# freshman97/LinTransUNet

Measured on AMD Instinct MI355X. Metric: 128^3 CT patches/sec (fwd+bwd), higher is better.
Workload: dtype bf16; 1 GPU; MaskTransUnet train step (fwd + 5-level loss + bwd), 128^3 single-channel patches, 2 per GPU, dropout 0.3, random-init weights; global_batch=2, parallelism=dp1, side_stream_concurrent=True, allreduce=none (1 rank)

## Files before the change

lintransunet_amd/csrc/conv_c16_ring.hip:

```cpp
#include "gemm_desc.h"
#include "lds_dma.h"

#define C16_PITCH 12
#define C16_HROWS 768
#define C16_HBUF (C16_HROWS * 32)
#define C16_STAGE (2 * C16_HBUF)
#define C16_BIAS (C16_STAGE + 4 * 4096)
#define C16_SMEM (C16_BIAS + 128)
#define C16_CENTER ((1 * 10 + 1) * C16_PITCH + 1)

template <bool FLIP>
__global__ void __launch_bounds__(256, 2) conv3_c16_ring_bf16_kernel(const HaloArgs a, int bricks) {
  extern __shared__ __attribute__((aligned(1024))) char smem[];
  const int tid = threadIdx.x, lane = tid & 63, wave = tid >> 6;
  const int li = lane & 31, lh = lane >> 5;
  const int nbh = (a.H + 3) / 4, nbw = (a.W + 7) / 8, nbd = (a.D + 7) / 8;
  const uint32_t lds0 = lds_addr(smem);
  const char* zsrc = reinterpret_cast<const char*>(ltu_zero_line) + (lane & 1) * 16;

  const int per = (bricks + (int)gridDim.x - 1) / (int)gridDim.x;
  const int b_first = (int)blockIdx.x * per;
  const int b_end = min(bricks, b_first + per);
  if (b_first >= b_end) return;

  bf16x8 wreg[27];
#pragma unroll
  for (int t = 0; t < 27; ++t) {
    uint4 v = make_uint4(0u, 0u, 0u, 0u);
    if (li < a.N) v = *reinterpret_cast<const uint4*>(reinterpret_cast<const uint16_t*>(a.w) + ((long long)li * 27 + t) * 16 + lh * 8);
    wreg[t] = __builtin_bit_cast(bf16x8, v);
  }
  const int prow = lane >> 1;
  const char* hbase[6];
  int hpos[6];
#pragma unroll
  for (int s = 0; s < 6; ++s) {
    const int row = (wave * 6 + s) * 32 + prow;
    const int hd = row % C16_PITCH, hw = (row / C16_PITCH) % 10, hh = row / (10 * C16_PITCH);
    const int c = ((lane & 1) ^ (hw & 1)) * 8;
    const bool s1 = c >= a.c0;
    const long long rel = ((long long)(hh - 1) * a.W + (hw - 1)) * a.D + (hd - 1);
    hbase[s] = s1 ? reinterpret_cast<const char*>(a.x1) + ((c - a.c0) + rel * a.lda1) * 2 : reinterpret_cast<const char*>(a.x0) + (c + rel * a.lda0) * 2;
    hpos[s] = hh | (hw << 8) | (hd << 16) | ((row < 6 * 10 * C16_PITCH && hd < 10 ? 1 : 0) << 24) | ((s1 ? 1 : 0) << 25);
  }
  struct Coord { int b, h0, w0, d0; };
  auto decompose = [&](int brick) {
    const Brick bk = split_brick(brick, nbh, nbw, nbd);
    return Coord{bk.b, bk.bh * 4, bk.bw * 8, bk.bd * 8};
  };
  auto advance = [&](Coord c) {
    c.d0 += 8;
    if (c.d0 >= nbd * 8) {
      c.d0 = 0; c.w0 += 8;
      if (c.w0 >= nbw * 8) {
        c.w0 = 0; c.h0 += 4;
        if (c.h0 >= nbh * 4) { c.h0 = 0; c.b += 1; }
      }
    }
    return c;
  };
  auto issue_halo = [&](const Coord& cc, int buf) {
    const int b = cc.b, h0 = cc.h0, w0 = cc.w0, d0 = cc.d0;
    const long long vox0 = (((long long)b * a.H + h0) * a.W + w0) * a.D + d0;
    const long long off0 = vox0 * a.lda0 * 2, off1 = vox0 * a.lda1 * 2;
    const uint32_t hb = lds0 + buf * C16_HBUF + wave * 6 * 1024;
    if (h0 >= 1 && h0 + 5 <= a.H && w0 >= 1 && w0 + 9 <= a.W && d0 >= 1 && d0 + 9 <= a.D) {
#pragma unroll
      for (int s = 0; s < 6; ++s) {
        const char* src = ((hpos[s] >> 24) & 1) ? hbase[s] + (((hpos[s] >> 25) & 1) ? off1 : off0) : zsrc;
        glds16(src, hb + s * 1024);
      }
      return;
    }
#pragma unroll
    for (int s = 0; s < 6; ++s) {
      const int h = h0 - 1 + (hpos[s] & 255), w = w0 - 1 + ((hpos[s] >> 8) & 255), d = d0 - 1 + ((hpos[s] >> 16) & 255);
      const bool in = ((hpos[s] >> 24) & 1) != 0 && (unsigned)h < (unsigned)a.H && (unsigned)w < (unsigned)a.W && (unsigned)d < (unsigned)a.D;
      const char* src = in ? hbase[s] + (((hpos[s] >> 25) & 1) ? off1 : off0) : zsrc;
      glds16(src, hb + s * 1024);
    }
  };

  const int hwl = li >> 3;
  int baseA[2][3];
#pragma unroll
  for (int i = 0; i < 2; ++i) {
    const int row0 = ((wave + 1) * 10 + (i * 4 + hwl + 1)) * C16_PITCH + (li & 7) + 1;
#pragma unroll
    for (int dwi = 0; dwi < 3; ++dwi) baseA[i][dwi] = (row0 - C16_CENTER) * 32 + ((lh ^ ((hwl + dwi) & 1)) << 4);
  }

  if (tid < 32) reinterpret_cast<float*>(smem + C16_BIAS)[tid] = (a.bias != nullptr && tid < a.N) ? a.bias[tid] : 0.f;
  char* obase[4];
  int opos[4];
#pragma unroll
  for (int it = 0; it < 4; ++it) {
    const int idx = it * 64 + lane, vox = idx >> 2, part = idx & 3;
    const int n = part * 8;
    const bool d1 = n >= a.n0;
    const long long rel = (long long)(vox >> 3) * a.D + (vox & 7);
    obase[it] = d1 ? reinterpret_cast<char*>(a.o1) + ((n - a.n0) + rel * a.ldo1) * 2 : reinterpret_cast<char*>(a.o0) + (n + rel * a.ldo0) * 2;
    opos[it] = (vox >> 3) | ((vox & 7) << 8) | ((n < a.N ? 1 : 0) << 16) | ((d1 ? 1 : 0) << 17);
  }
  char* const stage = smem + C16_STAGE + wave * 4096;

  auto store_brick = [&](const Coord& cc) {
    const int b = cc.b, h0 = cc.h0, w0 = cc.w0, d0 = cc.d0;
    const long long vox0 = ((((long long)b * a.H + h0 + wave) * a.W + w0) * a.D + d0);
    const long long off0 = vox0 * a.ldo0 * 2, off1 = vox0 * a.ldo1 * 2;
    const bool hok = h0 + wave < a.H;
    const bool whole = w0 + 8 <= a.W && d0 + 8 <= a.D;
#pragma unroll
    for (int it = 0; it < 4; ++it) {
      const int idx = it * 64 + lane, vox = idx >> 2, part = idx & 3;
      const uint4 v = *reinterpret_cast<const uint4*>(stage + vox * 64 + ((part ^ ((vox >> 1) & 3)) << 4));
      const int ow = opos[it] & 255, od = (opos[it] >> 8) & 255;
      if (hok && ((opos[it] >> 16) & 1) != 0 && (whole || (w0 + ow < a.W && d0 + od < a.D)))
        *reinterpret_cast<uint4*>(obase[it] + (((opos[it] >> 17) & 1) ? off1 : off0)) = v;
    }
  };
  Coord cur = decompose(b_first), prev = cur, next = advance(cur);
  issue_halo(cur, 0);
  int buf = 0;
  for (int brick = b_first; brick < b_end; ++brick) {
    ring_sync<0>();
    if (brick > b_first) store_brick(prev);
    if (brick + 1 < b_end) issue_halo(next, buf ^ 1);
    prev = cur; cur = next; next = advance(next);
    const int hoff = buf * C16_HBUF;
    int bA[2][3];
#pragma unroll
    for (int i = 0; i < 2; ++i)
#pragma unroll
      for (int dwi = 0; dwi < 3; ++dwi) bA[i][dwi] = baseA[i][dwi] + hoff;
    f32x16 acc[2];
#pragma unroll
    for (int i = 0; i < 2; ++i)
#pragma unroll
      for (int r = 0; r < 16; ++r) acc[i][r] = 0.f;
    auto load_frags = [&](auto TT, bf16x8 (&af)[2]) {
      constexpr int t = decltype(TT)::value;
      constexpr int th = t / 9, tw = (t / 3) % 3, td = t % 3;
      constexpr int dh = FLIP ? 1 - th : th - 1, dw = FLIP ? 1 - tw : tw - 1, dd = FLIP ? 1 - td : td - 1;
      constexpr int immA = (((dh * 10 + dw) * C16_PITCH + dd) + C16_CENTER) * 32;
#pragma unroll
      for (int i = 0; i < 2; ++i) af[i] = *reinterpret_cast<const bf16x8*>(smem + bA[i][dw + 1] + immA);
    };
    bf16x8 afA[2], afB[2];
    load_frags(std::integral_constant<int, 0>{}, afA);
    static_for<0, 14>([&](auto TP) {
      constexpr int t = decltype(TP)::value * 2;
      if constexpr (t + 1 < 27) load_frags(std::integral_constant<int, t + 1>{}, afB);
      __builtin_amdgcn_sched_barrier(0);
#pragma unroll
      for (int i = 0; i < 2; ++i) acc[i] = __builtin_amdgcn_mfma_f32_32x32x16_bf16(wreg[t], afA[i], acc[i], 0, 0, 0);
      __builtin_amdgcn_sched_barrier(0);
      if constexpr (t + 2 < 27) load_frags(std::integral_constant<int, t + 2>{}, afA);
      __builtin_amdgcn_sched_barrier(0);
      if constexpr (t + 1 < 27) {
#pragma unroll
        for (int i = 0; i < 2; ++i) acc[i] = __builtin_amdgcn_mfma_f32_32x32x16_bf16(wreg[t + 1], afB[i], acc[i], 0, 0, 0);
      }
      __builtin_amdgcn_sched_barrier(0);
    });
#pragma unroll
    for (int rr = 0; rr < 4; ++rr) {
      const float4 bv = *reinterpret_cast<const float4*>(smem + C16_BIAS + (8 * rr + 4 * lh) * 4);
#pragma unroll
      for (int i = 0; i < 2; ++i) {
        const int vox = i * 32 + li;
        uint2 pk;
        pk.x = pack_bf16x2(acc[i][4 * rr + 0] + bv.x, acc[i][4 * rr + 1] + bv.y);
        pk.y = pack_bf16x2(acc[i][4 * rr + 2] + bv.z, acc[i][4 * rr + 3] + bv.w);
        *reinterpret_cast<uint2*>(stage + vox * 64 + ((rr ^ ((vox >> 1) & 3)) << 4) + lh * 8) = pk;
      }
    }
    buf ^= 1;
  }
  store_brick(prev);
}

int launch_conv_c16_ring_bf16(const HaloArgs& a, hipStream_t st) {
  if (a.C != 16 || a.N > 32 || a.N % 8 || a.n0 % 8 || a.c0 % 8 || a.lda0 % 8 || a.lda1 % 8 || a.ldo0 % 8 || a.ldo1 % 8) return 1;
  if (a.H < 2 || a.W < 4 || a.D < 4 || a.part != nullptr) return 1;
  const long long bricks = (long long)a.B * ((a.H + 3) / 4) * ((a.W + 7) / 8) * ((a.D + 7) / 8);
  if (bricks >= (1LL << 31) || bricks < 128) return 1;
  static LtuDevOnce attr_once;
  if (attr_once.first()) {
    ltu_dyn_lds(&conv3_c16_ring_bf16_kernel<false>, C16_SMEM);
    ltu_dyn_lds(&conv3_c16_ring_bf16_kernel<true>, C16_SMEM);
  }
  const int want = ltu_knob_pos("LTU_C16_RING_BLOCKS", 512);
  const int nblk = (int)(bricks < want ? bricks : want);
  if (a.flip) hipLaunchKernelGGL(conv3_c16_ring_bf16_kernel<true>, dim3(nblk), dim3(256), C16_SMEM, st, a, (int)bricks);
  else hipLaunchKernelGGL(conv3_c16_ring_bf16_kernel<false>, dim3(nblk), dim3(256), C16_SMEM, st, a, (int)bricks);
  return ltu_check_launch();
}
```

lintransunet_amd/csrc/conv_halo.hip:

```cpp
#include "gemm_desc.h"
#include "lds_dma.h"

#define HALO_H 6
#define HALO_W 6
#define HALO_D 10
#define HALO_VOX (HALO_H * HALO_W * HALO_D)
#define LDH 40

template <int WN, int TN, int TS>
constexpr int halo_smem_bytes() {
  constexpr int BN = WN * TN * 32;
  constexpr int be = HALO_VOX * 32 + 2 * TS * BN * LDH, se = 128 * (BN + 8);
  return 2 * (be > se ? be : se);
}
template <int WM, int WN, int TM, int TN, int TS, int CC>
__global__ void __launch_bounds__(256) conv3_halo_bf16_kernel(const HaloArgs a) {
  static_assert(WM * TM == 4 && WM * WN == 4, "128-row brick on 4 waves");
  constexpr int BN = WN * TN * 32, NSTAGE = 27 / TS;
  constexpr int VPV = CC / 8, KS = CC / 16;
  constexpr int PD = CC == 16 ? 12 : HALO_D, VMASK = VPV - 1;
  constexpr int HALO_ELEMS = HALO_VOX * 32, B_ELEMS = 2 * TS * BN * LDH, LDC = BN + 8, STAGE_ELEMS = 128 * LDC;
  extern __shared__ __attribute__((aligned(16))) uint16_t smem[];
  uint16_t* halo = smem;
  uint16_t* Bs = smem + HALO_ELEMS;
// ... 565 lines not shown
      const float4 q = *reinterpret_cast<const float4*>(a.part + ((long long)z * M + v) * a.N + n);
      acc.x += q.x; acc.y += q.y; acc.z += q.z; acc.w += q.w;
    }
    uint2 pk;
    pk.x = pack_bf16x2(acc.x, acc.y);
    pk.y = pack_bf16x2(acc.z, acc.w);
    uint16_t* dst = n < a.n0 ? reinterpret_cast<uint16_t*>(a.o0) + v * a.ldo0 + n
                             : reinterpret_cast<uint16_t*>(a.o1) + v * a.ldo1 + (n - a.n0);
    *reinterpret_cast<uint2*>(dst) = pk;
  }
}

static int halo_split(long long bricks, int N, int C, int CC, int* cps) {
  if (N <= 32 && C <= 32) return 1;
  const int ntn = (N > 64 && bricks * cdiv(N, 128) >= 256) ? cdiv(N, 128) : (N > 32 ? cdiv(N, 64) : 1);
  const long long blocks = bricks * ntn;
  const int nchunk = (C + CC - 1) / CC;
  if (blocks >= ltu_knob_pos("LTU_HALO_SPLIT_BELOW", 200) || nchunk < 2) return 1;
  int want = (int)((512 + blocks - 1) / blocks);
  if (want > 8) want = 8;
  if (want > nchunk) want = nchunk;
  if (want < 2) return 1;
  *cps = (nchunk + want - 1) / want;
  return (nchunk + *cps - 1) / *cps;
}
static int halo_cc(int C, int c0) { return (C % 32 == 0 && c0 % 32 == 0) ? 32 : 16; }
long long conv_halo_ws_floats(int B, int H, int W, int D, int C, int N) {
  const long long bricks = (long long)B * ((H + 3) / 4) * ((W + 3) / 4) * ((D + 7) / 8);
  int cps = 0;
  if (conv_ring_splits(B, H, W, D, C, N)) return 8LL * B * H * W * D * N;
  const int ks = halo_split(bricks, N, C, halo_cc(C, C), &cps);
  return (ks > 1 || halo_split(bricks, N, C, 16, &cps) > 1) ? 8LL * B * H * W * D * N : 0;
}

int launch_conv_halo_bf16(HaloArgs a, hipStream_t st) {
  if (a.C % 8 || a.c0 % 8 || a.lda0 % 8 || a.lda1 % 8 || a.N % 4 || a.n0 % 4 || a.ldo0 % 4 || a.ldo1 % 4) return 1;
  if (a.H < 2 || a.W < 2 || a.D < 4) return 1;
  a.CC = (a.C % 32 == 0 && a.c0 % 32 == 0) ? 32 : 16;
  if (a.C % 16 != 0 && a.C != 8) return 1;
  if (a.c0 % a.CC != 0 && a.c0 != a.C) return 1;
  const long long bricks = (long long)a.B * ((a.H + 3) / 4) * ((a.W + 3) / 4) * ((a.D + 7) / 8);
  if (bricks >= (1LL << 31)) return 1;
#ifdef LTU_EXPERIMENTS
  a.no_xcd_order = ltu_knob("LTU_HALO_NO_XCD", 0);
#else
  a.no_xcd_order = 0;
#endif
  if (a.C == 32 && a.N <= 32 && !ltu_knob("LTU_NO_FC_RING", 0)) {
    const int hr = launch_conv_fc_ring_bf16(a, st);
    if (hr != 1) return hr;
  }
  if (a.C == 16 && a.N <= 32 && !ltu_knob("LTU_NO_C16_RING", 0)) {
    const int hr = launch_conv_c16_ring_bf16(a, st);
    if (hr != 1) return hr;
  }
  if (a.N <= 32 && a.C <= 32 && !ltu_knob("LTU_NO_HALO_WS", 0)) {
    int wsb = -1;
    wsb = ltu_knob_pos("LTU_HALO_WS_BLOCKS", 512);
    const unsigned nblk = (unsigned)(bricks < wsb ? bricks : wsb);
    if (ltu_knob("LTU_HALO_WR", a.C <= 16 ? 1 : 0)) {
      const int wrb = ltu_knob_pos("LTU_HALO_WR_BLOCKS", a.C > 16 ? 256 : 512);
      const unsigned nb = (unsigned)(bricks < wrb ? bricks : wrb);
      if (a.C > 16) hipLaunchKernelGGL((conv3_halo_wr_bf16_kernel<32>), dim3(nb), dim3(256), 0, st, a, (int)bricks);
      else hipLaunchKernelGGL((conv3_halo_wr_bf16_kernel<16>), dim3(nb), dim3(256), 0, st, a, (int)bricks);
      return ltu_check_launch();
    }
    if (a.C > 16) hipLaunchKernelGGL((conv3_halo_ws_bf16_kernel<32>), dim3(nblk), dim3(256), 0, st, a, (int)bricks);
    else hipLaunchKernelGGL((conv3_halo_ws_bf16_kernel<16>), dim3(nblk), dim3(256), 0, st, a, (int)bricks);
    return ltu_check_launch();
  }
  if ((a.C >= 64 || a.N > 32) && !ltu_knob("LTU_NO_CONV_RING", 0)) {
    a.ksplit = 1;
    const int hr = launch_conv_ring_bf16(a, st);
    if (hr == LTU_OK && a.ksplit > 1) {
      const long long M = (long long)a.B * a.H * a.W * a.D;
      long long blocks = (M * (a.N / 4) + 255) / 256;
      if (blocks > 2048) blocks = 2048;
      hipLaunchKernelGGL(conv_halo_fold_kernel, dim3((unsigned)blocks), dim3(256), 0, st, a, M);
      return ltu_check_launch();
    }
    if (hr != 1) return hr;
  }
  int cps = 0;
  a.ksplit = a.part != nullptr && !ltu_knob("LTU_NO_HALO_SPLIT", 0) ? halo_split(bricks, a.N, a.C, a.CC, &cps) : 1;
  a.cps = cps;
  if (a.ksplit < 2) a.part = nullptr;
  else if ((long long)a.ksplit * a.B * a.H * a.W * a.D * a.N > a.part_floats) return LTU_E_ARG;
  const unsigned gz = (unsigned)a.ksplit;
  const int chunks_per_wg = a.ksplit > 1 ? a.cps : (a.C + a.CC - 1) / a.CC;
  const bool deep = ltu_knob("LTU_HALO_DEEP", chunks_per_wg >= 4 ? 1 : 0) != 0;
#define HALO_LAUNCH1(WM, WN, TM, TN, TS, CCV)                                                                        \
  do {                                                                                                               \
    auto kern = &conv3_halo_bf16_kernel<WM, WN, TM, TN, TS, CCV>;                                                    \
    constexpr int bytes = halo_smem_bytes<WN, TN, TS>();                                                            \
    static LtuDevOnce once;                                                                                          \
    if (once.first()) ltu_dyn_lds(kern, bytes);                                                                      \
    hipLaunchKernelGGL(kern, grid, dim3(256), bytes, st, a);                                                         \
  } while (0)
#define HALO_LAUNCH(WM, WN, TM, TN, TS)                     \
  do {                                                      \
    if (a.CC == 32) HALO_LAUNCH1(WM, WN, TM, TN, TS, 32);   \
    else HALO_LAUNCH1(WM, WN, TM, TN, TS, 16);              \
  } while (0)
  if (a.N > 64 && bricks * cdiv(a.N, 128) >= 256) {
    dim3 grid((unsigned)bricks, cdiv(a.N, 128), gz);
    if (deep) HALO_LAUNCH(2, 2, 2, 2, 3);
// ... 791 lines not shown
```

lintransunet_amd/csrc/gemm.hip:

```cpp
#include <stdlib.h>

#include "gemm_desc.h"

template <typename TA>
__device__ __forceinline__ float4 gather_a(const IGemmArgs& g, bool row_ok, const RowCoord& rc, int k) {
  float4 z = make_float4(0.f, 0.f, 0.f, 0.f);
  if (!row_ok || k >= g.K) return z;
  const int slot = k / g.C;
  const int c = k - slot * g.C;
  const Tap tp = g.tap[slot];
  int h = rc.h * g.mh + tp.dh, w = rc.w * g.mw + tp.dw, d = rc.d * g.md + tp.dd;
  if ((unsigned)h >= (unsigned)g.sh || (unsigned)w >= (unsigned)g.sw || (unsigned)d >= (unsigned)g.sd) return z;
  int ph = g.sh, pw = g.sw, pd = g.sd;
  if (g.ups) {
    h >>= 1; w >>= 1; d >>= 1;
    ph >>= 1; pw >>= 1; pd >>= 1;
  }
  const long long vox = (((long long)rc.b * ph + h) * pw + w) * pd + d;
  if (c < g.c0) return Vec4<TA>::load(reinterpret_cast<const TA*>(g.a0) + vox * g.lda0 + c);
  return Vec4<TA>::load(reinterpret_cast<const TA*>(g.a1) + vox * g.lda1 + (c - g.c0));
}

__device__ __forceinline__ float4 gather_w(const IGemmArgs& g, int n, int k) {
  if (n >= g.N || k >= g.K) return make_float4(0.f, 0.f, 0.f, 0.f);
// ... 410 lines not shown
                                      ltu_stream_t s) {
  if (dtype != LTU_BF16) return LTU_E_DTYPE;
  const int rc = launch_tn_ring_group_bf16(jobs, njobs, blocks, ws, ws_floats, (hipStream_t)s);
  return rc == 1 ? LTU_E_SHAPE : rc;
}

static bool use_halo() {
  int v = -1;
  v = ltu_knob("LTU_NO_HALO", 0) ? 0 : 1;
  return v == 1;
}

static int conv_fwd_desc(IGemmArgs& g, int B, int Hi, int Wi, int Di, int C0, int C1, int Co, int sh, int sw, int sd,
                         int ups, int* Ho, int* Wo, int* Do) {
  if ((sh != 1 && sh != 2) || (sw != 1 && sw != 2) || (sd != 1 && sd != 2)) return LTU_E_ARG;
  if (C0 % 4 != 0 || C1 % 4 != 0 || C0 <= 0) return LTU_E_SHAPE;
  memset(&g, 0, sizeof(g));
  const int Hl = ups ? 2 * Hi : Hi, Wl = ups ? 2 * Wi : Wi, Dl = ups ? 2 * Di : Di;
  *Ho = (Hl - 1) / sh + 1; *Wo = (Wl - 1) / sw + 1; *Do = (Dl - 1) / sd + 1;
  g.nb = B; g.rh = *Ho; g.rw = *Wo; g.rd = *Do;
  g.M = (long long)B * g.rh * g.rw * g.rd;
  g.N = Co; g.C = C0 + C1; g.c0 = C0; g.K = 27 * g.C;
  g.lda0 = C0; g.lda1 = C1;
  g.nseg = 1; g.wrow = 27 * g.C;
  g.sh = Hl; g.sw = Wl; g.sd = Dl; g.ups = ups ? 1 : 0;
  g.mh = sh; g.mw = sw; g.md = sd;
  g.ntaps = 27;
  for (int t = 0; t < 27; ++t) g.tap[t] = Tap{(int8_t)(t / 9 - 1), (int8_t)((t / 3) % 3 - 1), (int8_t)(t % 3 - 1), (int8_t)t};
  g.out_identity = 1;
  g.n0 = Co;
  return LTU_OK;
}

extern "C" int ltu_conv3d_fwd(const void* x0, const void* x1, const void* wf, const float* bias, void* y, int B, int Hi,
                              int Wi, int Di, int C0, int C1, int Co, int sh, int sw, int sd, int ups, float* ws, long long ws_floats,
                              int dtype, ltu_stream_t s) {
  IGemmArgs g;
  int Ho, Wo, Do;
  int rc = conv_fwd_desc(g, B, Hi, Wi, Di, C0, C1, Co, sh, sw, sd, ups, &Ho, &Wo, &Do);
  if (rc) return rc;
  g.a0 = x0; g.a1 = x1 ? x1 : x0;
  g.w[0] = wf; g.bias[0] = bias;
  g.o0 = y; g.o1 = y; g.ldo0 = Co; g.ldo1 = Co;
  if (dtype == LTU_BF16) {
    if (sh == 1 && sw == 1 && sd == 1 && !ups && use_halo()) {
      HaloArgs a;
      memset(&a, 0, sizeof(a));
      a.x0 = x0; a.x1 = x1 ? x1 : x0; a.w = wf; a.bias = bias; a.o0 = y; a.o1 = y;
      a.B = B; a.H = Hi; a.W = Wi; a.D = Di;
      a.C = C0 + C1; a.c0 = C0; a.lda0 = C0; a.lda1 = C1 > 0 ? C1 : C0;
      a.N = Co; a.n0 = Co; a.ldo0 = Co; a.ldo1 = Co;
      a.part = ws; a.part_floats = ws_floats;
      const int hr = launch_conv_halo_bf16(a, (hipStream_t)s);
      if (hr != 1) return hr;
    }
    g.part = ws; g.part_floats = ws_floats;
    return launch_nt_bf16(g, (hipStream_t)s);
  }
  if (dtype != LTU_F32) return LTU_E_DTYPE;
  return launch_nt<float, float>(g, (hipStream_t)s);
}

extern "C" long long ltu_conv3d_ws_floats(int B, int H, int W, int D, int C, int Co) {
  const long long halo = conv_halo_ws_floats(B, H, W, D, C, Co), ig = igemm_nt_ws_floats((long long)B * H * W * D, Co, 27 * C);
  return halo > ig ? halo : ig;
}
extern "C" long long ltu_igemm_ws_floats(long long M, int N, int K) { return igemm_nt_ws_floats(M, N, K); }

extern "C" int ltu_conv3d_wgrad(const void* grad, const void* x0, const void* x1, float* dwf, float* db, int B, int Hi,
                                int Wi, int Di, int C0, int C1, int Co, int sh, int sw, int sd, int ups, int torch_co,
                                int torch_ci, float* ws, long long ws_floats, int dtype, ltu_stream_t s) {
  WGradArgs wa;
  memset(&wa, 0, sizeof(wa));
  int Ho, Wo, Do;
  int rc = conv_fwd_desc(wa.g, B, Hi, Wi, Di, C0, C1, Co, sh, sw, sd, ups, &Ho, &Wo, &Do);
  if (rc) return rc;
  if (Co % 4 != 0) return LTU_E_SHAPE;
  wa.g.a0 = x0; wa.g.a1 = x1 ? x1 : x0;
  wa.grad = grad; wa.ldg = Co; wa.dw = dwf; wa.db = db; wa.t_co = torch_co; wa.t_ci = torch_ci;
  wa.part = dtype == LTU_BF16 ? ws : nullptr; wa.part_floats = ws_floats; wa.nseg_w = 1;
  if (dtype == LTU_BF16 && ws != nullptr && sh == 1 && sw == 1 && sd == 1 && !ups && use_halo()) {
    WHaloArgs h;
    memset(&h, 0, sizeof(h));
    h.x0 = x0; h.x1 = x1 ? x1 : x0; h.grad = grad;
    h.B = B; h.H = Hi; h.W = Wi; h.D = Di;
    h.C = C0 + C1; h.c0 = C0; h.lda0 = C0; h.lda1 = C1 > 0 ? C1 : C0;
    h.N = Co; h.ldg = Co; h.part = ws; h.part_floats = ws_floats;
    int nsplit = 0;
    const int hr = launch_conv_wgrad_halo_bf16(h, &nsplit, (hipStream_t)s);
    if (hr == LTU_OK) {
      wa.npad = Co; wa.kpad = 27 * (C0 + C1);
      wa.bpart = ws + (long long)nsplit * wa.npad * wa.kpad;
      return launch_wgrad_reduce(wa, nsplit, (hipStream_t)s);
    }
    if (hr != 1) return hr;
  }
  if (dtype == LTU_BF16) return launch_tn_bf16(wa, (hipStream_t)s);
  if (dtype != LTU_F32) return LTU_E_DTYPE;
  return launch_tn<float>(wa, (hipStream_t)s);
}

extern "C" int ltu_conv3d_dgrad(const void* grad, const void* wd, void* dx0, void* dx1, int B, int Hl, int Wl, int Dl,
                                int C0, int C1, int Co, int sh, int sw, int sd, float* ws, long long ws_floats, int dtype, ltu_stream_t s) {
  if ((sh != 1 && sh != 2) || (sw != 1 && sw != 2) || (sd != 1 && sd != 2)) return LTU_E_ARG;
  if (Co % 4 != 0) return LTU_E_SHAPE;
  if (dtype == LTU_BF16 && sh == 1 && sw == 1 && sd == 1 && use_halo()) {
// ... 210 lines not shown
```

lintransunet_amd/csrc/gemm_desc.h:

```cpp
#pragma once
#include <stdlib.h>
#include "common.h"

struct Tap {
  int8_t dh, dw, dd, wt;
};

struct IGemmArgs {
  const void* a0;
  const void* a1;
  const void* w[3];
  const float* bias[3];
  void* o0;
  void* o1;
  long long M;
  int N, K;
  int C, c0;
  int lda0, lda1;
  int nseg;
  int wrow;
  int nb, rh, rw, rd;
  int sh, sw, sd, ups;
  int mh, mw, md;
  int ntaps;
// ... 51 lines not shown

struct TnGeom {
  int bn, bk, nn, nk, rows, nsplit;
  long long ws_floats;
};
static inline TnGeom tn_geometry(long long M, int N, int K, int brows) {
  TnGeom t;
  t.bk = 128;
  t.bn = N > 64 ? 128 : (N > 32 ? 64 : 32);
  t.nk = (K + t.bk - 1) / t.bk;
  t.nn = (N + t.bn - 1) / t.bn;
  int tn_want = -1, tn_min = -1;
  tn_want = ltu_knob_pos("LTU_TN_WANT", 1024);
  tn_min = ltu_knob_pos("LTU_TN_MINROWS", 128);
  long long want = tn_want / ((long long)t.nk * t.nn);
  if (want < 1) want = 1;
  long long rows = (M + want - 1) / want;
  if (rows < tn_min) rows = tn_min;
  rows = (rows + brows - 1) / brows * brows;
  t.rows = (int)rows;
  t.nsplit = (int)((M + rows - 1) / rows);
  t.ws_floats = (long long)t.nsplit * t.nn * t.bn * ((long long)t.nk * t.bk + 1);
  return t;
}


int launch_nt_bf16(const IGemmArgs& g, hipStream_t st);
int launch_tn_bf16(WGradArgs& wa, hipStream_t st);

struct HaloArgs {
  const void* x0;
  const void* x1;
  const void* w;
  const float* bias;
  void* o0;
  void* o1;
  int B, H, W, D;
  int C, c0, lda0, lda1;
  int N, n0, ldo0, ldo1;
  int flip;
  int CC;
  float* part;
  long long part_floats;
  int ksplit, cps;
  int no_xcd_order;
};
long long conv_halo_ws_floats(int B, int H, int W, int D, int C, int N);
int launch_conv_halo_bf16(HaloArgs a, hipStream_t st);
bool conv_ring_splits(int B, int H, int W, int D, int C, int N);
int launch_conv_ring_bf16(HaloArgs& a, hipStream_t st);
int launch_conv_fc_ring_bf16(const HaloArgs& a, hipStream_t st);
int launch_conv_c16_ring_bf16(const HaloArgs& a, hipStream_t st);

struct WHaloArgs {
  const void* x0;
  const void* x1;
  const void* grad;
  const void* grad1;
  int gn0, ldg1;
  int B, H, W, D;
  int C, c0, lda0, lda1;
  int N, ldg;
  int CC;
  int bricks, bricks_per_split;
  float* part;
  long long part_floats;
  float* bpart;
  int npad, kpad;
};
long long conv_wgrad_halo_ws_floats(int N, int K);
int launch_conv_wgrad_halo_bf16(WHaloArgs a, int* nsplit_out, hipStream_t st);
int launch_conv_wgrad_halo_ring_bf16(WHaloArgs a, int* nsplit_out, hipStream_t st);
int launch_wgrad_reduce(const WGradArgs& wa, int nsplit, hipStream_t st);

bool tn_ring_shape_ok(long long M, int N, int K);
long long tn_ring_ws_floats(long long M, int N, int K);
int launch_tn_ring_bf16(WGradArgs& wa, hipStream_t st, int* nsplit_out = nullptr);
int launch_nt_ring_bf16(const IGemmArgs& g, hipStream_t st);
long long tn_ring_group_ws_floats(const ltu_wgrad_job* jobs, int njobs, int blocks);
int launch_tn_ring_group_bf16(const ltu_wgrad_job* jobs, int njobs, int blocks, float* ws, long long ws_floats, hipStream_t st);

struct ClsEntry {
  int8_t dh, dw, dd, cls;
  int wbase;
};
struct ClassHaloArgs {
  const void* x;
  const void* w;
  const float* bias;
  void* o0;
  void* o1;
  int B, H, W, D;
  int C, lda;
  int N, n0, ldo0, ldo1;
  int Hh, Wh, Dh;
  int mh, mw, md;
  int wrow;
  int nent, ncls;
  int cls_begin[9];
  int8_t cls_p[8][4];
  ClsEntry ent[64];
};
int launch_conv_class_halo_bf16(const ClassHaloArgs& a, hipStream_t st);
int launch_pw_small_bf16(const void* x, int lda, const void* w, const float* bias, void* y, int ldy, long long M, int N, int K, int accumulate,
                         hipStream_t st);
int launch_sdgrad_ring_bf16(const void* grad, const void* wd, void* dx, int B, int Hl, int Wl, int Dl, int N, int Co, int sd, hipStream_t st);
// ... 19 lines not shown
```

Baseline: 162.2 patches/s.

## Generalize C16 ring conv into template; add C8 and stride-(2,2,1) ring kernels

Moves the 16-channel ring-buffered halo conv kernel into a templated header parameterized by channel count and stride. The template is then used for two new kernels: an 8-channel stride-1 conv that packs two taps per MFMA k-slice, and a 16-channel stride-(2,2,1) forward conv. The aim is to move these layer shapes off the generic halo/workspace and implicit-GEMM paths onto the LDS-DMA double-buffered ring kernel. The trade-offs are more templated kernel code and new dispatch conditions, with the new paths taken only above a minimum brick count.

```diff
diff --git a/lintransunet_amd/csrc/conv_c16_ring.hip b/lintransunet_amd/csrc/conv_c16_ring.hip
--- a/lintransunet_amd/csrc/conv_c16_ring.hip
+++ b/lintransunet_amd/csrc/conv_c16_ring.hip
@@ -1,183 +1,11 @@
-#include "gemm_desc.h"
-#include "lds_dma.h"
+#include "conv_ring488.h"
 
-#define C16_PITCH 12
-#define C16_HROWS 768
-#define C16_HBUF (C16_HROWS * 32)
-#define C16_STAGE (2 * C16_HBUF)
-#define C16_BIAS (C16_STAGE + 4 * 4096)
-#define C16_SMEM (C16_BIAS + 128)
-#define C16_CENTER ((1 * 10 + 1) * C16_PITCH + 1)
+#define C16_SMEM (Ring488<16, 1>::SMEM)
 
 template <bool FLIP>
 __global__ void __launch_bounds__(256, 2) conv3_c16_ring_bf16_kernel(const HaloArgs a, int bricks) {
   extern __shared__ __attribute__((aligned(1024))) char smem[];
-  const int tid = threadIdx.x, lane = tid & 63, wave = tid >> 6;
-  const int li = lane & 31, lh = lane >> 5;
-  const int nbh = (a.H + 3) / 4, nbw = (a.W + 7) / 8, nbd = (a.D + 7) / 8;
-  const uint32_t lds0 = lds_addr(smem);
-  const char* zsrc = reinterpret_cast<const char*>(ltu_zero_line) + (lane & 1) * 16;
-
-  const int per = (bricks + (int)gridDim.x - 1) / (int)gridDim.x;
-  const int b_first = (int)blockIdx.x * per;
-  const int b_end = min(bricks, b_first + per);
-  if (b_first >= b_end) return;
-
-  bf16x8 wreg[27];
-#pragma unroll
-  for (int t = 0; t < 27; ++t) {
-    uint4 v = make_uint4(0u, 0u, 0u, 0u);
-    if (li < a.N) v = *reinterpret_cast<const uint4*>(reinterpret_cast<const uint16_t*>(a.w) + ((long long)li * 27 + t) * 16 + lh * 8);
-    wreg[t] = __builtin_bit_cast(bf16x8, v);
-  }
-  const int prow = lane >> 1;
-  const char* hbase[6];
-  int hpos[6];
-#pragma unroll
-  for (int s = 0; s < 6; ++s) {
-    const int row = (wave * 6 + s) * 32 + prow;
-    const int hd = row % C16_PITCH, hw = (row / C16_PITCH) % 10, hh = row / (10 * C16_PITCH);
-    const int c = ((lane & 1) ^ (hw & 1)) * 8;
-    const bool s1 = c >= a.c0;
-    const long long rel = ((long long)(hh - 1) * a.W + (hw - 1)) * a.D + (hd - 1);
-    hbase[s] = s1 ? reinterpret_cast<const char*>(a.x1) + ((c - a.c0) + rel * a.lda1) * 2 : reinterpret_cast<const char*>(a.x0) + (c + rel * a.lda0) * 2;
-    hpos[s] = hh | (hw << 8) | (hd << 16) | ((row < 6 * 10 * C16_PITCH && hd < 10 ? 1 : 0) << 24) | ((s1 ? 1 : 0) << 25);
-  }
-  struct Coord { int b, h0, w0, d0; };
-  auto decompose = [&](int brick) {
-    const Brick bk = split_brick(brick, nbh, nbw, nbd);
-    return Coord{bk.b, bk.bh * 4, bk.bw * 8, bk.bd * 8};
-  };
-  auto advance = [&](Coord c) {
-    c.d0 += 8;
-    if (c.d0 >= nbd * 8) {
-      c.d0 = 0; c.w0 += 8;
-      if (c.w0 >= nbw * 8) {
-        c.w0 = 0; c.h0 += 4;
-        if (c.h0 >= nbh * 4) { c.h0 = 0; c.b += 1; }
-      }
-    }
-    return c;
-  };
-  auto issue_halo = [&](const Coord& cc, int buf) {
-    const int b = cc.b, h0 = cc.h0, w0 = cc.w0, d0 = cc.d0;
-    const long long vox0 = (((long long)b * a.H + h0) * a.W + w0) * a.D + d0;
-    const long long off0 = vox0 * a.lda0 * 2, off1 = vox0 * a.lda1 * 2;
-    const uint32_t hb = lds0 + buf * C16_HBUF + wave * 6 * 1024;
-    if (h0 >= 1 && h0 + 5 <= a.H && w0 >= 1 && w0 + 9 <= a.W && d0 >= 1 && d0 + 9 <= a.D) {
-#pragma unroll
-      for (int s = 0; s < 6; ++s) {
-        const char* src = ((hpos[s] >> 24) & 1) ? hbase[s] + (((hpos[s] >> 25) & 1) ? off1 : off0) : zsrc;
-        glds16(src, hb + s * 1024);
-      }
-      return;
-    }
-#pragma unroll
-    for (int s = 0; s < 6; ++s) {
-      const int h = h0 - 1 + (hpos[s] & 255), w = w0 - 1 + ((hpos[s] >> 8) & 255), d = d0 - 1 + ((hpos[s] >> 16) & 255);
-      const bool in = ((hpos[s] >> 24) & 1) != 0 && (unsigned)h < (unsigned)a.H && (unsigned)w < (unsigned)a.W && (unsigned)d < (unsigned)a.D;
-      const char* src = in ? hbase[s] + (((hpos[s] >> 25) & 1) ? off1 : off0) : zsrc;
-      glds16(src, hb + s * 1024);
-    }
-  };
-
-  const int hwl = li >> 3;
-  int baseA[2][3];
-#pragma unroll
-  for (int i = 0; i < 2; ++i) {
-    const int row0 = ((wave + 1) * 10 + (i * 4 + hwl + 1)) * C16_PITCH + (li & 7) + 1;
-#pragma unroll
-    for (int dwi = 0; dwi < 3; ++dwi) baseA[i][dwi] = (row0 - C16_CENTER) * 32 + ((lh ^ ((hwl + dwi) & 1)) << 4);
-  }
-
-  if (tid < 32) reinterpret_cast<float*>(smem + C16_BIAS)[tid] = (a.bias != nullptr && tid < a.N) ? a.bias[tid] : 0.f;
-  char* obase[4];
-  int opos[4];
-#pragma unroll
-  for (int it = 0; it < 4; ++it) {
-    const int idx = it * 64 + lane, vox = idx >> 2, part = idx & 3;
-    const int n = part * 8;
-    const bool d1 = n >= a.n0;
-    const long long rel = (long long)(vox >> 3) * a.D + (vox & 7);
-    obase[it] = d1 ? reinterpret_cast<char*>(a.o1) + ((n - a.n0) + rel * a.ldo1) * 2 : reinterpret_cast<char*>(a.o0) + (n + rel * a.ldo0) * 2;
-    opos[it] = (vox >> 3) | ((vox & 7) << 8) | ((n < a.N ? 1 : 0) << 16) | ((d1 ? 1 : 0) << 17);
-  }
-  char* const stage = smem + C16_STAGE + wave * 4096;
-
-  auto store_brick = [&](const Coord& cc) {
-    const int b = cc.b, h0 = cc.h0, w0 = cc.w0, d0 = cc.d0;
-    const long long vox0 = ((((long long)b * a.H + h0 + wave) * a.W + w0) * a.D + d0);
-    const long long off0 = vox0 * a.ldo0 * 2, off1 = vox0 * a.ldo1 * 2;
-    const bool hok = h0 + wave < a.H;
-    const bool whole = w0 + 8 <= a.W && d0 + 8 <= a.D;
-#pragma unroll
-    for (int it = 0; it < 4; ++it) {
-      const int idx = it * 64 + lane, vox = idx >> 2, part = idx & 3;
-      const uint4 v = *reinterpret_cast<const uint4*>(stage + vox * 64 + ((part ^ ((vox >> 1) & 3)) << 4));
-      const int ow = opos[it] & 255, od = (opos[it] >> 8) & 255;
-      if (hok && ((opos[it] >> 16) & 1) != 0 && (whole || (w0 + ow < a.W && d0 + od < a.D)))
-        *reinterpret_cast<uint4*>(obase[it] + (((opos[it] >> 17) & 1) ? off1 : off0)) = v;
-    }
-  };
-  Coord cur = decompose(b_first), prev = cur, next = advance(cur);
-  issue_halo(cur, 0);
-  int buf = 0;
-  for (int brick = b_first; brick < b_end; ++brick) {
-    ring_sync<0>();
-    if (brick > b_first) store_brick(prev);
-    if (brick + 1 < b_end) issue_halo(next, buf ^ 1);
-    prev = cur; cur = next; next = advance(next);
-    const int hoff = buf * C16_HBUF;
-    int bA[2][3];
-#pragma unroll
-    for (int i = 0; i < 2; ++i)
-#pragma unroll
-      for (int dwi = 0; dwi < 3; ++dwi) bA[i][dwi] = baseA[i][dwi] + hoff;
-    f32x16 acc[2];
-#pragma unroll
-    for (int i = 0; i < 2; ++i)
-#pragma unroll
-      for (int r = 0; r < 16; ++r) acc[i][r] = 0.f;
-    auto load_frags = [&](auto TT, bf16x8 (&af)[2]) {
-      constexpr int t = decltype(TT)::value;
-      constexpr int th = t / 9, tw = (t / 3) % 3, td = t % 3;
-      constexpr int dh = FLIP ? 1 - th : th - 1, dw = FLIP ? 1 - tw : tw - 1, dd = FLIP ? 1 - td : td - 1;
-      constexpr int immA = (((dh * 10 + dw) * C16_PITCH + dd) + C16_CENTER) * 32;
-#pragma unroll
-      for (int i = 0; i < 2; ++i) af[i] = *reinterpret_cast<const bf16x8*>(smem + bA[i][dw + 1] + immA);
-    };
-    bf16x8 afA[2], afB[2];
-    load_frags(std::integral_constant<int, 0>{}, afA);
-    static_for<0, 14>([&](auto TP) {
-      constexpr int t = decltype(TP)::value * 2;
-      if constexpr (t + 1 < 27) load_frags(std::integral_constant<int, t + 1>{}, afB);
-      __builtin_amdgcn_sched_barrier(0);
-#pragma unroll
-      for (int i = 0; i < 2; ++i) acc[i] = __builtin_amdgcn_mfma_f32_32x32x16_bf16(wreg[t], afA[i], acc[i], 0, 0, 0);
-      __builtin_amdgcn_sched_barrier(0);
-      if constexpr (t + 2 < 27) load_frags(std::integral_constant<int, t + 2>{}, afA);
-      __builtin_amdgcn_sched_barrier(0);
-      if constexpr (t + 1 < 27) {
-#pragma unroll
-        for (int i = 0; i < 2; ++i) acc[i] = __builtin_amdgcn_mfma_f32_32x32x16_bf16(wreg[t + 1], afB[i], acc[i], 0, 0, 0);
-      }
-      __builtin_amdgcn_sched_barrier(0);
-    });
-#pragma unroll
-    for (int rr = 0; rr < 4; ++rr) {
-      const float4 bv = *reinterpret_cast<const float4*>(smem + C16_BIAS + (8 * rr + 4 * lh) * 4);
-#pragma unroll
-      for (int i = 0; i < 2; ++i) {
-        const int vox = i * 32 + li;
-        uint2 pk;
-        pk.x = pack_bf16x2(acc[i][4 * rr + 0] + bv.x, acc[i][4 * rr + 1] + bv.y);
-        pk.y = pack_bf16x2(acc[i][4 * rr + 2] + bv.z, acc[i][4 * rr + 3] + bv.w);
-        *reinterpret_cast<uint2*>(stage + vox * 64 + ((rr ^ ((vox >> 1) & 3)) << 4) + lh * 8) = pk;
-      }
-    }
-    buf ^= 1;
-  }
-  store_brick(prev);
+  conv3_ring488_body<16, 1, FLIP>(a, bricks, smem);
 }
 
 int launch_conv_c16_ring_bf16(const HaloArgs& a, hipStream_t st) {
diff --git a/lintransunet_amd/csrc/conv_c8_ring.hip b/lintransunet_amd/csrc/conv_c8_ring.hip
--- /dev/null
+++ b/lintransunet_amd/csrc/conv_c8_ring.hip
@@ -0,0 +1,26 @@
+#include "conv_ring488.h"
+
+#define C8_SMEM (Ring488<8, 1>::SMEM)
+
+template <bool FLIP>
+__global__ void __launch_bounds__(256, 2) conv3_c8_ring_bf16_kernel(const HaloArgs a, int bricks) {
+  extern __shared__ __attribute__((aligned(1024))) char smem[];
+  conv3_ring488_body<8, 1, FLIP>(a, bricks, smem);
+}
+
+int launch_conv_c8_ring_bf16(const HaloArgs& a, hipStream_t st) {
+  if (a.C != 8 || a.c0 < 8 || a.N > 32 || a.N % 8 || a.n0 % 8 || a.lda0 % 8 || a.ldo0 % 8 || a.ldo1 % 8) return 1;
+  if (a.H < 2 || a.W < 4 || a.D < 4) return 1;
+  const long long bricks = (long long)a.B * ((a.H + 3) / 4) * ((a.W + 7) / 8) * ((a.D + 7) / 8);
+  if (bricks >= (1LL << 31) || bricks < ltu_knob_pos("LTU_C8_RING_MIN_BRICKS", 1024)) return 1;
+  static LtuDevOnce attr_once;
+  if (attr_once.first()) {
+    ltu_dyn_lds(&conv3_c8_ring_bf16_kernel<false>, C8_SMEM);
+    ltu_dyn_lds(&conv3_c8_ring_bf16_kernel<true>, C8_SMEM);
+  }
+  const int want = ltu_knob_pos("LTU_C8_RING_BLOCKS", 512);
+  const int nblk = (int)(bricks < want ? bricks : want);
+  if (a.flip) hipLaunchKernelGGL(conv3_c8_ring_bf16_kernel<true>, dim3(nblk), dim3(256), C8_SMEM, st, a, (int)bricks);
+  else hipLaunchKernelGGL(conv3_c8_ring_bf16_kernel<false>, dim3(nblk), dim3(256), C8_SMEM, st, a, (int)bricks);
+  return ltu_check_launch();
+}
diff --git a/lintransunet_amd/csrc/conv_halo.hip b/lintransunet_amd/csrc/conv_halo.hip
--- a/lintransunet_amd/csrc/conv_halo.hip
+++ b/lintransunet_amd/csrc/conv_halo.hip
@@ -641,6 +641,10 @@
   }
   if (a.C == 16 && a.N <= 32 && !ltu_knob("LTU_NO_C16_RING", 0)) {
     const int hr = launch_conv_c16_ring_bf16(a, st);
+    if (hr != 1) return hr;
+  }
+  if (a.C == 8 && a.N <= 32 && !ltu_knob("LTU_NO_C8_RING", 0)) {
+    const int hr = launch_conv_c8_ring_bf16(a, st);
     if (hr != 1) return hr;
   }
   if (a.N <= 32 && a.C <= 32 && !ltu_knob("LTU_NO_HALO_WS", 0)) {
diff --git a/lintransunet_amd/csrc/conv_ring488.h b/lintransunet_amd/csrc/conv_ring488.h
--- /dev/null
+++ b/lintransunet_amd/csrc/conv_ring488.h
@@ -0,0 +1,234 @@
+#pragma once
+#include "gemm_desc.h"
+#include "lds_dma.h"
+
+template <int C, int S>
+struct Ring488 {
+  static_assert((C == 8 && S == 1) || (C == 16 && (S == 1 || S == 2)), "conv_ring488.h: C = 8 or 16 at stride 1, C = 16 at stride (2,2,1)");
+  static constexpr int BH = S == 1 ? 4 : 2;
+  static constexpr int NT = S == 1 ? 2 : 1;
+  static constexpr int HH = S * BH + 3 - S, HW = S * 8 + 3 - S, HD = 10;
+  static constexpr int PITCH = S == 1 ? 12 : 10;
+  static constexpr int ROWB = C * 2;
+  static constexpr int ROWS = C == 16 ? HH * HW * PITCH : 720;
+  static constexpr int PROWS = 1024 / ROWB;
+  static constexpr int NP = (ROWS + 4 * PROWS - 1) / (4 * PROWS);
+  static constexpr int HBUF = NP * 4 * 1024;
+  static constexpr int STAGE = 2 * HBUF;
+  static constexpr int STAGEW = NT * 2048;
+  static constexpr int BIAS = STAGE + 4 * STAGEW;
+  static constexpr int SMEM = BIAS + 128;
+  static constexpr int NW = C == 16 ? 27 : 14;
+};
+__host__ __device__ constexpr int c8_row(int hh, int hw, int hd) { return (hh >> 1) * 240 + hw * 24 + (hh & 1) * 12 + hd; }
+
+template <int C, int S, bool FLIP>
+__device__ __forceinline__ void conv3_ring488_body(const HaloArgs& a, int bricks, char* smem) {
+  using R = Ring488<C, S>;
+  static_assert(S == 1 || !FLIP, "the strided form is forward only");
+  const int tid = threadIdx.x, lane = tid & 63, wave = tid >> 6;
+  const int li = lane & 31, lh = lane >> 5;
+  const int plane = S == 1 ? wave : wave >> 1;
+  const int wt0 = S == 1 ? 0 : (wave & 1) * 4;
+  const int Ho = (a.H - 1) / S + 1, Wo = (a.W - 1) / S + 1, Do = a.D;
+  const int nbh = (Ho + R::BH - 1) / R::BH, nbw = (Wo + 7) / 8, nbd = (Do + 7) / 8;
+  const uint32_t lds0 = lds_addr(smem);
+  const char* zsrc = reinterpret_cast<const char*>(ltu_zero_line) + (lane & 1) * 16;
+
+  const int per = (bricks + (int)gridDim.x - 1) / (int)gridDim.x;
+  const int b_first = (int)blockIdx.x * per;
+  const int b_end = min(bricks, b_first + per);
+  if (b_first >= b_end) return;
+
+  bf16x8 wreg[R::NW];
+#pragma unroll
+  for (int t = 0; t < R::NW; ++t) {
+    uint4 v = make_uint4(0u, 0u, 0u, 0u);
+    if constexpr (C == 16) {
+      if (li < a.N) v = *reinterpret_cast<const uint4*>(reinterpret_cast<const uint16_t*>(a.w) + ((long long)li * 27 + t) * 16 + lh * 8);
+    } else {
+      const int q = 2 * t + lh;
+      if (li < a.N && q < 27) v = *reinterpret_cast<const uint4*>(reinterpret_cast<const uint16_t*>(a.w) + ((long long)li * 27 + (FLIP ? 26 - q : q)) * 8);
+    }
+    wreg[t] = __builtin_bit_cast(bf16x8, v);
+  }
+  const char* hbase[R::NP];
+  int hpos[R::NP];
+#pragma unroll
+  for (int s = 0; s < R::NP; ++s) {
+    if constexpr (C == 16) {
+      const int row = (wave * R::NP + s) * 32 + (lane >> 1);
+      const int hd = row % R::PITCH, hw = (row / R::PITCH) % R::HW, hh = row / (R::HW * R::PITCH);
+      const int c = ((lane & 1) ^ ((hw >> (S - 1)) & 1)) * 8;
+      const bool s1 = c >= a.c0;
+      const long long rel = ((long long)(hh - 1) * a.W + (hw - 1)) * a.D + (hd - 1);
+      hbase[s] = s1 ? reinterpret_cast<const char*>(a.x1) + ((c - a.c0) + rel * a.lda1) * 2 : reinterpret_cast<const char*>(a.x0) + (c + rel * a.lda0) * 2;
+      hpos[s] = hh | (hw << 8) | (hd << 16) | ((row < R::ROWS && hd < R::HD ? 1 : 0) << 24) | ((s1 ? 1 : 0) << 25);
+    } else {
+      const int row = (wave * R::NP + s) * 64 + lane;
+      const int hw = (row % 240) / 24, r2 = row % 24;
+      const int hd = r2 % 12, hh = 2 * (row / 240) + r2 / 12;
+      const long long rel = ((long long)(hh - 1) * a.W + (hw - 1)) * a.D + (hd - 1);
+      hbase[s] = reinterpret_cast<const char*>(a.x0) + rel * a.lda0 * 2;
+      hpos[s] = hh | (hw << 8) | (hd << 16) | ((row < R::ROWS && hd < R::HD ? 1 : 0) << 24);
+    }
+  }
+  struct Coord { int b, h0, w0, d0; };
+  auto decompose = [&](int brick) {
+    const Brick bk = split_brick(brick, nbh, nbw, nbd);
+    return Coord{bk.b, bk.bh * R::BH, bk.bw * 8, bk.bd * 8};
+  };
+  auto advance = [&](Coord c) {
+    c.d0 += 8;
+    if (c.d0 >= nbd * 8) {
+      c.d0 = 0; c.w0 += 8;
+      if (c.w0 >= nbw * 8) {
+        c.w0 = 0; c.h0 += R::BH;
+        if (c.h0 >= nbh * R::BH) { c.h0 = 0; c.b += 1; }
+      }
+    }
+    return c;
+  };
+  auto issue_halo = [&](const Coord& cc, int buf) {
+    const int b = cc.b, h0 = S * cc.h0, w0 = S * cc.w0, d0 = cc.d0;
+    const long long vox0 = (((long long)b * a.H + h0) * a.W + w0) * a.D + d0;
+    const long long off0 = vox0 * a.lda0 * 2, off1 = vox0 * a.lda1 * 2;
+    const uint32_t hb = lds0 + buf * R::HBUF + wave * R::NP * 1024;
+    if (h0 >= 1 && h0 + R::HH - 1 <= a.H && w0 >= 1 && w0 + R::HW - 1 <= a.W && d0 >= 1 && d0 + R::HD - 1 <= a.D) {
+#pragma unroll
+      for (int s = 0; s < R::NP; ++s) {
+        const char* src = ((hpos[s] >> 24) & 1) ? hbase[s] + (((hpos[s] >> 25) & 1) ? off1 : off0) : zsrc;
+        glds16(src, hb + s * 1024);
+      }
+      return;
+    }
+#pragma unroll
+    for (int s = 0; s < R::NP; ++s) {
+      const int h = h0 - 1 + (hpos[s] & 255), w = w0 - 1 + ((hpos[s] >> 8) & 255), d = d0 - 1 + ((hpos[s] >> 16) & 255);
+      const bool in = ((hpos[s] >> 24) & 1) != 0 && (unsigned)h < (unsigned)a.H && (unsigned)w < (unsigned)a.W && (unsigned)d < (unsigned)a.D;
+      const char* src = in ? hbase[s] + (((hpos[s] >> 25) & 1) ? off1 : off0) : zsrc;
+      glds16(src, hb + s * 1024);
+    }
+  };
+
+  const int hwl = li >> 3;
+  int baseA[R::NT][3];
+#pragma unroll
+  for (int i = 0; i < R::NT; ++i) {
+#pragma unroll
+    for (int k = 0; k < 3; ++k) {
+      if constexpr (C == 16) {
+        const int row0 = (S * plane * R::HW + S * (wt0 + i * 4 + hwl)) * R::PITCH + (li & 7);
+        baseA[i][k] = row0 * 32 + ((lh ^ ((hwl + (S == 1 ? k : k >> 1)) & 1)) << 4);
+      } else {
+        baseA[i][k] = c8_row(plane + k, i * 4 + hwl, li & 7) * 16;
+      }
+    }
+  }
+
+  if (tid < 32) reinterpret_cast<float*>(smem + R::BIAS)[tid] = (a.bias != nullptr && tid < a.N) ? a.bias[tid] : 0.f;
+  char* obase[2 * R::NT];
+  int opos[2 * R::NT];
+#pragma unroll
+  for (int it = 0; it < 2 * R::NT; ++it) {
+    const int idx = it * 64 + lane, vox = idx >> 2, part = idx & 3;
+    const int n = part * 8;
+    const bool d1 = n >= a.n0;
+    const int ow = wt0 + (vox >> 3), od = vox & 7;
+    const long long rel = (long long)ow * Do + od;
+    obase[it] = d1 ? reinterpret_cast<char*>(a.o1) + ((n - a.n0) + rel * a.ldo1) * 2 : reinterpret_cast<char*>(a.o0) + (n + rel * a.ldo0) * 2;
+    opos[it] = ow | (od << 8) | ((n < a.N ? 1 : 0) << 16) | ((d1 ? 1 : 0) << 17);
+  }
+  char* const stage = smem + R::STAGE + wave * R::STAGEW;
+
+  auto store_brick = [&](const Coord& cc) {
+    const int b = cc.b, h0 = cc.h0, w0 = cc.w0, d0 = cc.d0;
+    const long long vox0 = ((((long long)b * Ho + h0 + plane) * Wo + w0) * Do + d0);
+    const long long off0 = vox0 * a.ldo0 * 2, off1 = vox0 * a.ldo1 * 2;
+    const bool hok = h0 + plane < Ho;
+    const bool whole = w0 + 8 <= Wo && d0 + 8 <= Do;
+#pragma unroll
+    for (int it = 0; it < 2 * R::NT; ++it) {
+      const int idx = it * 64 + lane, vox = idx >> 2, part = idx & 3;
+      const uint4 v = *reinterpret_cast<const uint4*>(stage + vox * 64 + ((part ^ ((vox >> 1) & 3)) << 4));
+      const int ow = opos[it] & 255, od = (opos[it] >> 8) & 255;
+      if (hok && ((opos[it] >> 16) & 1) != 0 && (whole || (w0 + ow < Wo && d0 + od < Do)))
+        *reinterpret_cast<uint4*>(obase[it] + (((opos[it] >> 17) & 1) ? off1 : off0)) = v;
+    }
+  };
+  Coord cur = decompose(b_first), prev = cur, next = advance(cur);
+  issue_halo(cur, 0);
+  int buf = 0;
+  for (int brick = b_first; brick < b_end; ++brick) {
+    ring_sync<0>();
+    if (brick > b_first) store_brick(prev);
+    if (brick + 1 < b_end) issue_halo(next, buf ^ 1);
+    prev = cur; cur = next; next = advance(next);
+    const int hoff = buf * R::HBUF;
+    int bA[R::NT][3];
+#pragma unroll
+    for (int i = 0; i < R::NT; ++i)
+#pragma unroll
+      for (int k = 0; k < 3; ++k) bA[i][k] = baseA[i][k] + hoff;
+    f32x16 acc[R::NT];
+#pragma unroll
+    for (int i = 0; i < R::NT; ++i)
+#pragma unroll
+      for (int r = 0; r < 16; ++r) acc[i][r] = 0.f;
+    auto load_frags = [&](auto TT, bf16x8 (&af)[R::NT]) {
+      constexpr int t = decltype(TT)::value;
+      if constexpr (C == 16) {
+        constexpr int q = FLIP ? 26 - t : t;
+        constexpr int th = q / 9, tw = (q / 3) % 3, td = q % 3;
+        constexpr int immA = ((th * R::HW + tw) * R::PITCH + td) * 32;
+#pragma unroll
+        for (int i = 0; i < R::NT; ++i) af[i] = *reinterpret_cast<const bf16x8*>(smem + bA[i][tw] + immA);
+      } else {
+        constexpr int q0 = 2 * t, q1 = 2 * t + 1 < 27 ? 2 * t + 1 : 26;
+        constexpr int imm0 = ((q0 / 3) % 3 * 24 + q0 % 3) * 16, imm1 = ((q1 / 3) % 3 * 24 + q1 % 3) * 16;
+#pragma unroll
+        for (int i = 0; i < R::NT; ++i) {
+          const int ad = lh ? bA[i][q1 / 9] + imm1 : bA[i][q0 / 9] + imm0;
+          bf16x8 v = *reinterpret_cast<const bf16x8*>(smem + ad);
+          if constexpr (2 * t + 1 >= 27) {
+            const bf16x8 z = __builtin_bit_cast(bf16x8, make_uint4(0u, 0u, 0u, 0u));
+            v = lh ? z : v;
+          }
+          af[i] = v;
+        }
+      }
+    };
+    constexpr int NW = R::NW;
+    bf16x8 afA[R::NT], afB[R::NT];
+    load_frags(std::integral_constant<int, 0>{}, afA);
+    static_for<0, (NW + 1) / 2>([&](auto TP) {
+      constexpr int t = decltype(TP)::value * 2;
+      if constexpr (t + 1 < NW) load_frags(std::integral_constant<int, t + 1>{}, afB);
+      __builtin_amdgcn_sched_barrier(0);
+#pragma unroll
+      for (int i = 0; i < R::NT; ++i) acc[i] = __builtin_amdgcn_mfma_f32_32x32x16_bf16(wreg[t], afA[i], acc[i], 0, 0, 0);
+      __builtin_amdgcn_sched_barrier(0);
+      if constexpr (t + 2 < NW) load_frags(std::integral_constant<int, t + 2>{}, afA);
+      __builtin_amdgcn_sched_barrier(0);
+      if constexpr (t + 1 < NW) {
+#pragma unroll
+        for (int i = 0; i < R::NT; ++i) acc[i] = __builtin_amdgcn_mfma_f32_32x32x16_bf16(wreg[t + 1], afB[i], acc[i], 0, 0, 0);
+      }
+      __builtin_amdgcn_sched_barrier(0);
+    });
+#pragma unroll
+    for (int rr = 0; rr < 4; ++rr) {
+      const float4 bv = *reinterpret_cast<const float4*>(smem + R::BIAS + (8 * rr + 4 * lh) * 4);
+#pragma unroll
+      for (int i = 0; i < R::NT; ++i) {
+        const int vox = i * 32 + li;
+        uint2 pk;
+        pk.x = pack_bf16x2(acc[i][4 * rr + 0] + bv.x, acc[i][4 * rr + 1] + bv.y);
+        pk.y = pack_bf16x2(acc[i][4 * rr + 2] + bv.z, acc[i][4 * rr + 3] + bv.w);
+        *reinterpret_cast<uint2*>(stage + vox * 64 + ((rr ^ ((vox >> 1) & 3)) << 4) + lh * 8) = pk;
+      }
+    }
+    buf ^= 1;
+  }
+  store_brick(prev);
+}
diff --git a/lintransunet_amd/csrc/conv_s221_ring.hip b/lintransunet_amd/csrc/conv_s221_ring.hip
--- /dev/null
+++ b/lintransunet_amd/csrc/conv_s221_ring.hip
@@ -0,0 +1,22 @@
+#include "conv_ring488.h"
+
+#define S221_SMEM (Ring488<16, 2>::SMEM)
+
+__global__ void __launch_bounds__(256, 2) conv3_s221_ring_bf16_kernel(const HaloArgs a, int bricks) {
+  extern __shared__ __attribute__((aligned(1024))) char smem[];
+  conv3_ring488_body<16, 2, false>(a, bricks, smem);
+}
+
+int launch_conv_s221_ring_bf16(const HaloArgs& a, hipStream_t st) {
+  if (a.C != 16 || a.N > 32 || a.N % 8 || a.n0 % 8 || a.c0 % 8 || a.lda0 % 8 || a.lda1 % 8 || a.ldo0 % 8 || a.ldo1 % 8 || a.flip) return 1;
+  if (a.H < 2 || a.W < 4 || a.D < 4) return 1;
+  const int Ho = (a.H - 1) / 2 + 1, Wo = (a.W - 1) / 2 + 1;
+  const long long bricks = (long long)a.B * ((Ho + 1) / 2) * ((Wo + 7) / 8) * ((a.D + 7) / 8);
+  if (bricks >= (1LL << 31) || bricks < ltu_knob_pos("LTU_S221_RING_MIN_BRICKS", 1024)) return 1;
+  static LtuDevOnce attr_once;
+  if (attr_once.first()) ltu_dyn_lds(&conv3_s221_ring_bf16_kernel, S221_SMEM);
+  const int want = ltu_knob_pos("LTU_S221_RING_BLOCKS", 512);
+  const int nblk = (int)(bricks < want ? bricks : want);
+  hipLaunchKernelGGL(conv3_s221_ring_bf16_kernel, dim3(nblk), dim3(256), S221_SMEM, st, a, (int)bricks);
+  return ltu_check_launch();
+}
diff --git a/lintransunet_amd/csrc/gemm.hip b/lintransunet_amd/csrc/gemm.hip
--- a/lintransunet_amd/csrc/gemm.hip
+++ b/lintransunet_amd/csrc/gemm.hip
@@ -486,6 +486,16 @@
       a.N = Co; a.n0 = Co; a.ldo0 = Co; a.ldo1 = Co;
       a.part = ws; a.part_floats = ws_floats;
       const int hr = launch_conv_halo_bf16(a, (hipStream_t)s);
+      if (hr != 1) return hr;
+    }
+    if (sh == 2 && sw == 2 && sd == 1 && !ups && C0 + C1 == 16 && Co <= 32 && use_halo() && !ltu_knob("LTU_NO_S221_RING", 0)) {
+      HaloArgs a;
+      memset(&a, 0, sizeof(a));
+      a.x0 = x0; a.x1 = x1 ? x1 : x0; a.w = wf; a.bias = bias; a.o0 = y; a.o1 = y;
+      a.B = B; a.H = Hi; a.W = Wi; a.D = Di;
+      a.C = C0 + C1; a.c0 = C0; a.lda0 = C0; a.lda1 = C1 > 0 ? C1 : C0;
+      a.N = Co; a.n0 = Co; a.ldo0 = Co; a.ldo1 = Co;
+      const int hr = launch_conv_s221_ring_bf16(a, (hipStream_t)s);
       if (hr != 1) return hr;
     }
     g.part = ws; g.part_floats = ws_floats;
diff --git a/lintransunet_amd/csrc/gemm_desc.h b/lintransunet_amd/csrc/gemm_desc.h
--- a/lintransunet_amd/csrc/gemm_desc.h
+++ b/lintransunet_amd/csrc/gemm_desc.h
@@ -127,6 +127,9 @@
 int launch_conv_fc_ring_bf16(const HaloArgs& a, hipStream_t st);
 int launch_conv_c16_ring_bf16(const HaloArgs& a, hipStream_t st);
 
+int launch_conv_c8_ring_bf16(const HaloArgs& a, hipStream_t st);
+int launch_conv_s221_ring_bf16(const HaloArgs& a, hipStream_t st);
+
 struct WHaloArgs {
   const void* x0;
   const void* x1;
```

Result: no change. 162.6 patches/s (median of 4 runs) (+0.2%).
